# soedinglab/plass

Hardware: AMD Instinct MI355X
Metric: read-overlaps/s per assembly iteration (higher is better)
Workload: dtype u8/u64 (integer hash, byte compare; f32 ratios)

## Files before the change

### plass_amd/csrc/asm_rules.hpp

```cpp
#pragma once
#include <cmath>
#include <cstdlib>
#if defined(__HIPCC__)
#define PLASSHIP_AR_HD __host__ __device__ __forceinline__
#else
#define PLASSHIP_AR_HD static inline __attribute__((always_inline))
#endif
namespace plasship {

struct AlnCoords { int qStart, qEnd, dbStart, dbEnd; };
struct DiagSpan { bool hit = false; unsigned qo = 0, to = 0, len = 0; };

PLASSHIP_AR_HD int alnLengthOf(int qStart, int qEnd, int dbStart, int dbEnd) {
    const int aq = (qStart == -1) ? 0 : qStart, ad = (dbStart == -1) ? 0 : dbStart;
    const int dq = abs(qEnd - aq), dd = abs(dbEnd - ad);
    return (dq > dd ? dq : dd) + 1;
}
PLASSHIP_AR_HD int rawScoreOfBits(int bitScore, double ln2, double logK, double lambda) {
    return (int) (fma((double) bitScore, ln2, logK) / lambda + 0.5);
}
template <typename S> PLASSHIP_AR_HD int scorePerCol100(S score, unsigned alnLen) {
    const float scorePerCol = (float) score / (float) ((double) alnLen + 0.5);
    return (int) (scorePerCol * 100);
}
// ... 6 lines not shown
}
PLASSHIP_AR_HD AlnCoords alnOnDiagonal(int diag, int startPos, int endPos) {
    const int dist = abs(diag);
    AlnCoords c;
    if (diag >= 0) { c.qStart = startPos + dist; c.qEnd = endPos + dist; c.dbStart = startPos; c.dbEnd = endPos; }
    else { c.qStart = startPos; c.qEnd = endPos; c.dbStart = startPos + dist; c.dbEnd = endPos + dist; }
    return c;
}
PLASSHIP_AR_HD float rescoredSeqId(int ids, int qStart, int qEnd) {
    return (float) ids / ((float) qEnd - (float) qStart);
}
PLASSHIP_AR_HD bool isBranchType(int qStart, int qEnd, unsigned qLen, int dbStart, int dbEnd, unsigned dbLen) {
    const bool notBoth = !(dbStart == 0 && qStart == 0);
    const bool rightStart = dbStart == 0 && (dbEnd != (int) dbLen - 1);
    const bool leftStart = qStart == 0 && (qEnd != (int) qLen - 1);
    return (rightStart || leftStart) && notBoth;
}
PLASSHIP_AR_HD unsigned rightFragLen(unsigned tLen, int dbEnd) { return tLen - ((unsigned) dbEnd + 1); }
PLASSHIP_AR_HD bool canExtendRight(unsigned fragR, int qEnd, unsigned qLen) { return fragR > 0 && (unsigned) qEnd == (qLen - 1); }
PLASSHIP_AR_HD bool canExtendLeft(int dbStart, int dbEnd, unsigned tLen) { return dbStart > 0 && (unsigned) dbEnd == (tLen - 1); }
PLASSHIP_AR_HD bool deferredRight(unsigned fragR, int qEnd, unsigned qLen, unsigned rightOff) {
    return fragR > rightOff && (unsigned) qEnd == (qLen - 1) && rightOff > 0;
}
PLASSHIP_AR_HD bool deferredLeft(int dbStart, int dbEnd, unsigned tLen, unsigned leftOff) {
    return dbStart > (int) leftOff && (unsigned) dbEnd == (tLen - 1) && leftOff > 0;
}
PLASSHIP_AR_HD AlnCoords mirrorReverseHit(int qStart, int qEnd, int dbStart, int dbEnd, unsigned dbLen) {
    AlnCoords c;
    c.qStart = qEnd; c.qEnd = qStart;
    c.dbStart = (int) (dbLen - (unsigned) dbEnd - 1); c.dbEnd = (int) (dbLen - (unsigned) dbStart - 1);
    return c;
}

}
```

### plass_amd/csrc/assemble.hip

```cpp
#include "common.hpp"
#include "device_utils.hpp"
#include "posterior_class.hpp"
#include "ref_rules.hpp"
#include "asm_rules.hpp"
#include "host_util.hpp"
#include <algorithm>
#include <memory>
#include <cstring>

namespace plasship {

struct Item {
    uint32_t target; int32_t score; uint32_t alnLength; float seqId;
    int32_t qStart, qEnd; uint32_t qLen; int32_t dbStart, dbEnd; uint32_t dbLen;
    uint32_t state;
    uint32_t pad;
};

struct AsmArgs {
    SeqView s;
    const uint64_t *qoff; const AlnRec *recs;
    Item *items;
    const uint64_t *arenaOff;
    const uint32_t *leftCap;
// ... 1162 lines not shown
                deferred = 0;
            }
            while (deferred) {
                const int dl = __ffsll((long long) deferred) - 1;
                deferred &= deferred - 1;
                const int dqs = __shfl(xQStart, dl, G), dds = __shfl(xDbStart, dl, G);
                const char *tSeq = a.s.data + __shfl(xTOff, dl, G);
                const unsigned tLen = __shfl(xTLen, dl, G);
                const int diag = (int) ((unsigned) dqs + leftOff) - dds;
                const Rescored rs = rescoreOnDiagonalG<G>(qs, querySeqLen, tSeq, tLen, diag, smat, gl);
                nResc += (gl == 0); nRescRes += (gl == 0) ? rs.diagonalLen : 0;
                const AlnCoords c = alnOnDiagonal(diag, rs.startPos, rs.endPos);
                const float seqId = rescoredSeqId(rs.idExcl, c.qStart, c.qEnd);
                if (gl == dl) {
                    xQLen = querySeqLen; xDbLen = tLen; xAlnLen = rs.diagonalLen; xScore = scorePerCol100(rs.score, rs.diagonalLen);
                    xQStart = c.qStart; xQEnd = c.qEnd; xDbStart = c.dbStart; xDbEnd = c.dbEnd;
                    xState = (seqId >= a.seqIdThr) ? 0u : 2u;
                }
            }
            inQueue = (uint32_t) __popcll(groupBallot<G>(xState == 0));
        }
        if (couldExtend) {
            if (gl == 0) { atomicOr(&a.flags[id], 0x20u); a.newLen[id] = (uint32_t) curLen; a.newStart[id] = aoff + curStart; nExt++; }
        }
    }
    nExt = waveReduceSumU64(nExt); nResc = waveReduceSumU64(nResc); nRescRes = waveReduceSumU64(nRescRes); nAln = waveReduceSumU64(nAln); nQRes = waveReduceSumU64(nQRes);
    if (laneId() == 0) {
        if (nExt) atomicAdd(&a.stats[0], nExt); if (nResc) atomicAdd(&a.stats[1], nResc); if (nRescRes) atomicAdd(&a.stats[2], nRescRes);
        const int tier = (G <= 16) ? 0 : 1;
        if (nAln) { atomicAdd(&a.stats[3 + 3 * tier], nAln); atomicAdd(&a.stats[4 + 3 * tier], nQRes); atomicAdd(&a.stats[5 + 3 * tier], nRescRes); }
    }
}

__global__ __launch_bounds__(256) void arenaSumKernel(const AlnRec *__restrict__ recs, uint64_t nAln, uint64_t maxSeqLen, unsigned long long *__restrict__ qSum,
                                                      unsigned long long *__restrict__ qSumAa, uint32_t *__restrict__ qCan, int mirror) {
    const int lane = laneId();
    for (uint64_t i = (uint64_t) blockIdx.x * blockDim.x + threadIdx.x; i < nAln; i += (uint64_t) gridDim.x * blockDim.x) {
        const AlnRec r = recs[i];
        const uint32_t id = r.query;
        uint32_t add = 0, addAa = 0; bool can = false;
        if (r.target != id && r.accepted) {
            add = (uint32_t) r.dbLen; addAa = (uint32_t) r.dbLen / 3 + 2;
            AlnCoords c; c.qStart = r.qStart; c.qEnd = r.qEnd; c.dbStart = r.dbStart; c.dbEnd = r.dbEnd;
            if (mirror && c.qStart > c.qEnd) c = mirrorReverseHit(r.qStart, r.qEnd, r.dbStart, r.dbEnd, (unsigned) r.dbLen);
            if (isBranchType(c.qStart, c.qEnd, (unsigned) r.qLen, c.dbStart, c.dbEnd, (unsigned) r.dbLen)) {
                if (c.dbStart == 0) can = canExtendRight(rightFragLen((unsigned) r.dbLen, c.dbEnd), c.qEnd, (unsigned) r.qLen);
                else if (c.qStart == 0) can = canExtendLeft(c.dbStart, c.dbEnd, (unsigned) r.dbLen) && ((uint64_t) r.qLen + (uint64_t) c.dbStart < maxSeqLen);
            }
        }
        const unsigned long long act = __ballot(1);
        const uint32_t prevId = (uint32_t) __shfl_up((int) id, 1, 64);
        const bool head = lane == 0 || prevId != id;
        const unsigned long long heads = __ballot(head), cans = __ballot(can);
        const int segStart = 63 - __clzll((long long) (heads & (lane == 63 ? ~0ULL : ((2ULL << lane) - 1ULL))));
        const unsigned long long later = lane == 63 ? 0ULL : (heads & ~((2ULL << lane) - 1ULL));
        const int segEnd = (later ? __ffsll((long long) later) - 1 : (int) __popcll(act)) - 1;
#pragma unroll
        for (int d = 1; d < 64; d <<= 1) {
            const uint32_t t = (uint32_t) __shfl_up((int) add, d, 64), ta = (uint32_t) __shfl_up((int) addAa, d, 64);
            if (lane - d >= segStart) { add += t; addAa += ta; }
        }
        if (lane == segEnd) {
            const unsigned long long seg = (segEnd == 63 ? ~0ULL : ((2ULL << segEnd) - 1ULL)) & ~((1ULL << segStart) - 1ULL);
            if (add) atomicAdd(&qSum[id], (unsigned long long) add);
            if (qSumAa && addAa) atomicAdd(&qSumAa[id], (unsigned long long) addAa);
            if (cans & seg) atomicOr(&qCan[id], 1u);
        }
    }
}
constexpr int N_TIERS = 5;
constexpr uint8_t TIER_NARROW = 4, TIER_NONE = 0xFF;
__global__ void arenaSizeKernel(SeqView s, const uint64_t *__restrict__ qoff, const unsigned long long *__restrict__ qSum, const unsigned long long *__restrict__ qSumAa,
                                const uint32_t *__restrict__ qCan, uint32_t *__restrict__ leftCap,
                                uint64_t *__restrict__ bytes, int nuclTiers, uint64_t threadBytes,
                                uint8_t *__restrict__ tierOf,
                                const uint32_t *__restrict__ aaLen, uint32_t *__restrict__ aaLeftCap, uint64_t *__restrict__ aaBytes) {
    for (uint32_t id = blockIdx.x * blockDim.x + threadIdx.x; id < s.n; id += gridDim.x * blockDim.x) {
        int tier = -1;
        const uint64_t sum = qSum[id], sumAa = aaBytes ? qSumAa[id] : 0;
        const bool can = qCan[id] != 0;
        leftCap[id] = (uint32_t) std::min<uint64_t>(sum, 0xFFFFFFFFull);
        const uint64_t slice = (sum && can) ? (2 * sum + s.len[id] + 40) : 0;
        bytes[id] = slice;
        if (aaBytes) { aaLeftCap[id] = (uint32_t) std::min<uint64_t>(sumAa, 0xFFFFFFFFull); aaBytes[id] = (sum && can) ? (2 * sumAa + aaLen[id] + 8) : 0; }
        if (sum && can) { const uint64_t h = qoff[id + 1] - qoff[id]; tier = nuclTiers ? ((h <= 256 && slice <= threadBytes) ? 0 : 1) : (h <= 8 ? (int) TIER_NARROW : (h <= 16 ? 0 : (h <= 32 ? 1 : (h <= 64 ? 2 : 3)))); }
        tierOf[id] = (tier < 0) ? TIER_NONE : (uint8_t) tier;
    }
}
static_assert(SCAN_TILE < (1 << 12) && N_TIERS * 12 <= 64 && SCAN_BLOCK == 256, "tier counters of a tile: 12-bit fields of one 64-bit word");
__device__ __forceinline__ unsigned long long tierField(uint8_t t) { return (t < N_TIERS) ? (1ull << (12 * t)) : 0ull; }
__device__ __forceinline__ uint64_t loadTierBytes(const uint8_t *__restrict__ tierOf, uint32_t n, uint64_t base) {
    static_assert(SCAN_ITEMS == 8, "eight tier bytes per thread");
    if (base + 8 <= n) return *reinterpret_cast<const uint64_t *>(tierOf + base);
    uint64_t w = ~0ull;
    for (int k = 0; k < 8; k++) if (base + k < n) w = (w & ~(0xFFull << (8 * k))) | ((uint64_t) tierOf[base + k] << (8 * k));
    return w;
}
__global__ __launch_bounds__(SCAN_BLOCK) void tierCountKernel(const uint8_t *__restrict__ tierOf, uint32_t n, uint64_t *__restrict__ partial, uint32_t nTiles) {
    __shared__ unsigned long long wsum[SCAN_BLOCK / WAVE];
// ... 480 lines not shown
    if (al->nQueries != db->n) { setError("plasship_assemble: alignment list does not belong to the DB"); return PLASSHIP_ERR_ARG; }
    PH_ENTER(ctx);
    hipStream_t st = ctx->stream;
    const uint32_t N = (uint32_t) db->n;
    if (nucl) { const int rcS = finishSelfAlns(ctx, al); if (rcS) return rcS; }
    const uint64_t nLines = al->nSlots;
    DevBuf dLeftCap, dBytes, dArenaOff, dTmp, dItems, dFlags, dNewLen, dNewStart, dMat, dStats, dArena;
    const size_t tmpBytes = exclusiveScanTmpBytes((size_t) N + 2);
    if (dLeftCap.alloc(((size_t) N + 1) * 4) != hipSuccess || dBytes.alloc(((size_t) N + 1) * 8) != hipSuccess || dArenaOff.alloc(((size_t) N + 2) * 8) != hipSuccess ||
        dTmp.alloc(tmpBytes) != hipSuccess || dItems.alloc(std::max<uint64_t>(nLines, 1) * sizeof(Item)) != hipSuccess || dFlags.alloc(((size_t) N + 1) * 4) != hipSuccess ||
        dNewLen.alloc(((size_t) N + 1) * 4) != hipSuccess || dNewStart.alloc(((size_t) N + 1) * 8) != hipSuccess || dMat.alloc(123 * 123) != hipSuccess || dStats.alloc(128) != hipSuccess) {
        setError("plasship_assemble: out of device memory"); return PLASSHIP_ERR_DEVICE;
    }
    PH_CHECK(hipMemsetAsync(dFlags.p, 0, ((size_t) N + 1) * 4, st));
    PH_CHECK(hipMemsetAsync(dNewLen.p, 0, ((size_t) N + 1) * 4, st));
    PH_CHECK(hipMemsetAsync(dStats.p, 0, 128, st));
    PH_CHECK(hipMemcpyAsync(dMat.p, asciiSubMat(nucl), 123 * 123, hipMemcpyHostToDevice, st));
    { const int rcOL = ensureOffLen(ctx, db); if (rcOL) return rcOL; }
    const SeqView sv = db->view();
    PH_CHECK(hipEventRecord(ctx->ev[0], st));
    const uint32_t nTiles = (uint32_t) (((size_t) N + SCAN_TILE - 1) / SCAN_TILE);
    DevBuf dBigList, dMidList, dMid32List, dSmallList, dNarrowList, dTierOf, dTierPart, dAaLeftCap, dAaBytes, dAaArenaOff, dAaArena, dAaNewLen, dAaNewStart;
    if (guided && (dAaLeftCap.alloc(((size_t) N + 1) * 4) != hipSuccess || dAaBytes.alloc(((size_t) N + 1) * 8) != hipSuccess || dAaArenaOff.alloc(((size_t) N + 2) * 8) != hipSuccess ||
                   dAaNewLen.alloc(((size_t) N + 1) * 4) != hipSuccess || dAaNewStart.alloc(((size_t) N + 1) * 8) != hipSuccess)) { setError("plasship_assemble: out of device memory"); return PLASSHIP_ERR_DEVICE; }
    if (guided) PH_CHECK(hipMemsetAsync(dAaNewLen.p, 0, ((size_t) N + 1) * 4, st));
    if (dBigList.alloc(((size_t) N + 1) * 4) != hipSuccess || dMidList.alloc(((size_t) N + 1) * 4) != hipSuccess || dMid32List.alloc(((size_t) N + 1) * 4) != hipSuccess ||
        dSmallList.alloc(((size_t) N + 1) * 4) != hipSuccess || (!nucl && dNarrowList.alloc(((size_t) N + 1) * 4) != hipSuccess) || dTierOf.alloc((size_t) N + 8) != hipSuccess ||
        dTierPart.alloc(((size_t) N_TIERS * (nTiles + 1) + 1) * 8) != hipSuccess) { setError("plasship_assemble: out of device memory"); return PLASSHIP_ERR_DEVICE; }
    DevBuf dQSum, dQSumAa, dQCan;
    if (dQSum.alloc(((size_t) N + 1) * 8) != hipSuccess || dQCan.alloc(((size_t) N + 1) * 4) != hipSuccess || (guided && dQSumAa.alloc(((size_t) N + 1) * 8) != hipSuccess)) { setError("plasship_assemble: out of device memory"); return PLASSHIP_ERR_DEVICE; }
    PH_CHECK(hipMemsetAsync(dQSum.p, 0, ((size_t) N + 1) * 8, st));
    PH_CHECK(hipMemsetAsync(dQCan.p, 0, ((size_t) N + 1) * 4, st));
    if (guided) PH_CHECK(hipMemsetAsync(dQSumAa.p, 0, ((size_t) N + 1) * 8, st));
    if (nLines) hipLaunchKernelGGL(arenaSumKernel, dim3((unsigned) std::min<uint64_t>((nLines + 255) / 256, (uint64_t) ctx->numCU * 32)), dim3(256), 0, st, al->d_recs.as<AlnRec>(), (uint64_t) nLines,
                                       (uint64_t) par->max_seq_len, dQSum.as<unsigned long long>(), guided ? dQSumAa.as<unsigned long long>() : (unsigned long long *) nullptr, dQCan.as<uint32_t>(),
                                       (nucl && !guided) ? 1 : 0);
    if (N) hipLaunchKernelGGL(arenaSizeKernel, dim3(std::min<uint32_t>((N + 255) / 256, 8192)), dim3(256), 0, st, sv, al->d_qoff.as<uint64_t>(), (const unsigned long long *) dQSum.as<unsigned long long>(),
                              (const unsigned long long *) dQSumAa.as<unsigned long long>(), (const uint32_t *) dQCan.as<uint32_t>(), dLeftCap.as<uint32_t>(), dBytes.as<uint64_t>(), nucl ? 1 : 0, (uint64_t) 1 << 30,
                              dTierOf.as<uint8_t>(),
                              guided ? aaDb->d_len.as<uint32_t>() : (const uint32_t *) nullptr, dAaLeftCap.as<uint32_t>(), guided ? dAaBytes.as<uint64_t>() : (uint64_t *) nullptr);
    if (guided && exclusiveScanU64(st, dAaBytes.as<uint64_t>(), dAaArenaOff.as<uint64_t>(), N, dTmp.p, tmpBytes)) { setError("plasship_assemble: scan failed"); return PLASSHIP_ERR_DEVICE; }
    PH_CHECK(hipMemsetAsync(dTierPart.p, 0, ((size_t) N_TIERS * (nTiles + 1) + 1) * 8, st));
    if (nTiles) hipLaunchKernelGGL(tierCountKernel, dim3(nTiles), dim3(SCAN_BLOCK), 0, st, (const uint8_t *) dTierOf.as<uint8_t>(), N, dTierPart.as<uint64_t>(), nTiles);
    if (exclusiveScanU64(st, dTierPart.as<uint64_t>(), dTierPart.as<uint64_t>(), (size_t) N_TIERS * (nTiles + 1), dTmp.p, tmpBytes)) { setError("plasship_assemble: scan failed"); return PLASSHIP_ERR_DEVICE; }
    {
        TierLists tl;
        tl.list[0] = dSmallList.as<uint32_t>(); tl.list[1] = dMid32List.as<uint32_t>(); tl.list[2] = dMidList.as<uint32_t>(); tl.list[3] = dBigList.as<uint32_t>();
        tl.list[TIER_NARROW] = dNarrowList.as<uint32_t>();
        if (nTiles) hipLaunchKernelGGL(tierListKernel, dim3(nTiles), dim3(SCAN_BLOCK), 0, st, (const uint8_t *) dTierOf.as<uint8_t>(), N, (const uint64_t *) dTierPart.as<uint64_t>(), nTiles, tl);
    }
    if (exclusiveScanU64(st, dBytes.as<uint64_t>(), dArenaOff.as<uint64_t>(), N, dTmp.p, tmpBytes)) { setError("plasship_assemble: scan failed"); return PLASSHIP_ERR_DEVICE; }
    uint64_t arenaBytes = 0, aaArenaBytes = 0;
    uint64_t rowStart[N_TIERS + 1] = {};
    if (guided) PH_CHECK(hipMemcpyAsync(&aaArenaBytes, dAaArenaOff.as<uint64_t>() + N, 8, hipMemcpyDeviceToHost, st));
    PH_CHECK(hipMemcpyAsync(&arenaBytes, dArenaOff.as<uint64_t>() + N, 8, hipMemcpyDeviceToHost, st));
    PH_CHECK(hipMemcpy2DAsync(rowStart, 8, dTierPart.p, (size_t) (nTiles + 1) * 8, 8, N_TIERS + 1, hipMemcpyDeviceToHost, st));
    PH_CHECK(plasship::streamSync(st));
    uint32_t cnts[N_TIERS];
    for (int t = 0; t < N_TIERS; t++) cnts[t] = (uint32_t) (rowStart[t + 1] - rowStart[t]);
    if (dArena.alloc(arenaBytes + 64) != hipSuccess || (guided && dAaArena.alloc(aaArenaBytes + 64) != hipSuccess)) {
        size_t fr = 0, tt = 0; (void) hipMemGetInfo(&fr, &tt);
        setError("plasship_assemble: out of device memory for the extension arena (" + std::to_string(arenaBytes) + " bytes; device free " + std::to_string(fr) + " of " + std::to_string(tt) + ")"); return PLASSHIP_ERR_DEVICE;
    }
    HostEvaluer ev(nucl, db->residues);
    AsmArgs a; memset(&a, 0, sizeof(a));
    a.s = sv; a.qoff = al->d_qoff.as<uint64_t>(); a.recs = al->d_recs.as<AlnRec>(); a.items = dItems.as<Item>(); a.arenaOff = dArenaOff.as<uint64_t>();
    a.leftCap = dLeftCap.as<uint32_t>(); a.arena = dArena.as<char>(); a.flags = dFlags.as<uint32_t>(); a.newLen = dNewLen.as<uint32_t>(); a.newStart = dNewStart.as<uint64_t>();
// ... 172 lines not shown
```

### plass_amd/csrc/common.hpp

```cpp
#pragma once
#include <hip/hip_runtime.h>
#include <cstdint>
#include <cstddef>
#include <cstdio>
#include <atomic>
#include <functional>
#include <memory>
#include <mutex>
#include <string>
#include <vector>
#include "../../include/plasship.h"

namespace plasship {

void setError(const std::string &msg);
hipError_t streamSync(hipStream_t st);
}
struct plasship_seqdb; struct plasship_ctx;
namespace plasship {
int ensureOffLen(plasship_ctx *ctx, const plasship_seqdb *db);
std::string hipErrStr(hipError_t e, const char *what, const char *file, int line);

#define PH_CHECK(call)                                                                   \
    do {                                                                                 \
// ... 136 lines not shown

struct plasship_cands {
    bool reverseCapable = false;
    size_t nQueries = 0;
    uint64_t nHits = 0;
    uint64_t nNonSelf = 0;
    plasship::DevBuf d_qoff;
    plasship::DevBuf d_hits;
    std::vector<uint8_t> h_present;
};

struct plasship_clusters {
    size_t n = 0;
    uint64_t nClusters = 0;
    uint64_t dbGen = 0;
    plasship::DevBuf d_pairs;
    plasship::DevBuf d_repOf;
};

struct plasship_alns {
    size_t nQueries = 0;
    uint64_t nLines = 0;
    uint64_t nSlots = 0;
    bool sparse = false;
    mutable bool selfPending = false;
    plasship_rescore_params rsPar = {};
    bool rsSameDB = false; int rsReverseCapable = 0;
    bool nucl = false;
    bool addBacktrace = false;
    uint64_t dbResidues = 0;
    int gappedOpen = 0, gappedExtend = 0;
    plasship::DevBuf d_qoff;
    plasship::DevBuf d_recs;
    const plasship_seqdb *qdb = nullptr, *tdb = nullptr;
};

namespace plasship {
inline const plasship_comm *commOf(const plasship_ctx *ctx) { return ctx->hasComm ? &ctx->comm : nullptr; }
inline uint64_t ownedBegin(uint64_t n, int r, int world) { return ((uint64_t) r * n + (uint64_t) world - 1) / (uint64_t) world; }
int commAllgatherHost(plasship_ctx *ctx, const void *send, void *recv, uint64_t bytesPerRank);
int commAllReduceSumU64(plasship_ctx *ctx, uint64_t *v, size_t n);
int commAllReduceMaxU64(plasship_ctx *ctx, uint64_t *v, size_t n);
int commAllReduceMinU64(plasship_ctx *ctx, uint64_t *v, size_t n);
int commAgreeOk(plasship_ctx *ctx, bool ok, const char *what);
int commFinish(plasship_ctx *ctx, int rc);
int commAlltoallvRecords(plasship_ctx *ctx, const void *dSend, const uint64_t *sendCount, size_t recordBytes, DevBuf &recv,
                         uint64_t *recvTotal, uint64_t slackRecords, uint64_t *allTotal = nullptr);
int commAllgathervBytes(plasship_ctx *ctx, const void *dSend, uint64_t sendBytes, DevBuf &recv, std::vector<uint64_t> &recvBytes);
int commAllgathervBytesKnown(plasship_ctx *ctx, const void *dSend, uint64_t sendBytes, DevBuf &recv, const std::vector<uint64_t> &recvBytes);
int packedCopyOf(plasship_ctx *ctx, const plasship_seqdb *db, std::unique_ptr<plasship_seqdb> &out);
int buildOutputDB(plasship_ctx *ctx, const plasship_seqdb *db, const uint32_t *dFlags, const uint32_t *dNewLen, const uint64_t *dNewStart,
                  const char *dArena, int keepTarget, void *dTmp, size_t tmpBytes, plasship_seqdb **out,
                  const void *dExtra = nullptr, void *hExtra = nullptr, size_t extraBytes = 0, hipEvent_t doneEvent = nullptr, bool noAppend = false);
int stagedUpload(plasship_ctx *ctx, void *dDst, uint64_t total, const std::function<void(char *, uint64_t, uint64_t)> &produce,
                 uint64_t chunk = 0, const std::function<int(uint64_t)> *enqueued = nullptr);
int stagedDownload(plasship_ctx *ctx, const void *dSrc, uint64_t total, const std::function<bool(const char *, uint64_t, uint64_t)> &consume);
void *ctxPinnedTable(plasship_ctx *ctx, size_t bytes);
int stagedCopyToDevice(plasship_ctx *ctx, void *dDst, const void *hSrc, uint64_t bytes);
int stagedCopyToHost(plasship_ctx *ctx, void *hDst, const void *dSrc, uint64_t bytes);
int deviceKeysDiffer(plasship_ctx *ctx, const uint32_t *a, const uint32_t *b, size_t n, bool *differ);
int compactCsr(plasship_ctx *ctx, const char *what, const uint64_t *dInQoff, uint64_t nQ, const void *dRecs, size_t recBytes, const uint32_t *dKeep,
               uint64_t nRecs, uint64_t nKept, DevBuf &outQoff, DevBuf &outRecs);
int denseAlnsCopy(plasship_ctx *ctx, const plasship_alns *a, DevBuf &qoffBuf, DevBuf &recsBuf, const uint64_t **qoff, const AlnRec **recs);
int finishSelfAlns(plasship_ctx *ctx, const plasship_alns *a, const uint32_t *dQueryList = nullptr, uint32_t nQueryList = 0);
}
```

### plass_amd/csrc/core.hip

```cpp
#include "common.hpp"
#include "host_util.hpp"
#include "device_utils.hpp"
#include <algorithm>
#include <atomic>
#include <condition_variable>
#include <thread>
#include <memory>
#include <chrono>
#include <cstdio>
#include <cstdlib>
#include <cstring>
#include <map>
#include <mutex>
#include <numeric>
#include <unordered_map>
#include <unistd.h>

namespace plasship {
namespace {
std::mutex g_poolMu;
constexpr size_t POOL_ALIGN = 256;
struct FreeRange { size_t size; hipStream_t stream; bool mixed; };
struct Slab { char *base; size_t size; size_t used; std::map<size_t, FreeRange> free; };
struct DevicePool { std::vector<Slab> slabs; size_t total = 0; };
// ... 114 lines not shown
    std::lock_guard<std::mutex> g(g_poolMu);
    auto it = g_poolLive.find(p);
    if (it == g_poolLive.end()) { (void) hipFree(p); return; }
    const PoolLive lv = it->second;
    g_poolLive.erase(it);
    Slab &sl = g_pools[lv.device].slabs[lv.slab];
    sl.used -= lv.size;
    size_t off = lv.off, size = lv.size; hipStream_t stream = lv.stream; bool mixed = (tl_poolStream != nullptr && tl_poolStream != lv.stream);
    auto nx = sl.free.lower_bound(off);
    if (nx != sl.free.end() && off + size == nx->first) {
        if (nx->second.mixed || nx->second.stream != stream) mixed = !(nx->second.stream == nullptr && !nx->second.mixed) || mixed;
        size += nx->second.size; nx = sl.free.erase(nx);
    }
    if (nx != sl.free.begin()) {
        auto pv = std::prev(nx);
        if (pv->first + pv->second.size == off) {
            if (pv->second.mixed || pv->second.stream != stream) mixed = !(pv->second.stream == nullptr && !pv->second.mixed) || mixed;
            off = pv->first; size += pv->second.size; sl.free.erase(pv);
        }
    }
    sl.free[off] = FreeRange{size, stream, mixed};
}
void poolTrim() {
    std::lock_guard<std::mutex> g(g_poolMu);
    trimLocked(-1);
}
static thread_local std::string g_err;
int tuneInt(const char *name, int dflt) {
    char key[96]; snprintf(key, sizeof(key), "PLASSHIP_TUNE_%s", name);
    const char *e = getenv(key); const int v = e ? atoi(e) : 0;
    return v > 0 ? v : dflt;
}
static const char *const TUNE_NAMES[] = {"AGGWAVE", "AGGWAVE_CAP", "ASMQ", "ASMQ_CAP", "ROWTIER", "KMCACHE", "FORCE_LONG", "CYC_PASSES", "CYCSKIP", "SHARD_EXTRACT",
                                         "FASTA_CHUNK_MB", "DBHEAP", "DBHEAP_GB", "LAZY_SELF", "FASTQ_CHUNK_KB", "PART_BITS", "GROUP_SHAPE"};
static void reportUnknownTunes() {
    static const char PREFIX[] = "PLASSHIP_TUNE_";
    for (char **e = environ; e && *e; e++) {
        if (strncmp(*e, PREFIX, sizeof(PREFIX) - 1) != 0) continue;
        const char *x = *e + sizeof(PREFIX) - 1, *eq = strchr(x, '=');
        const std::string name(x, eq ? (size_t) (eq - x) : strlen(x));
        bool known = false;
        for (const char *k : TUNE_NAMES) known = known || name == k;
        if (!known) fprintf(stderr, "[plasship] PLASSHIP_TUNE_%s is not a switch of this build (ignored)\n", name.c_str());
    }
}
bool traceOn() { static const bool v = getenv("PLASSHIP_TRACE") != nullptr; return v; }
void setError(const std::string &msg) { g_err = msg; }
static std::atomic<unsigned long long> g_hostSyncs(0);
thread_local int tl_watchRank = -1, tl_watchWorld = 1;
thread_local const char *tl_watchLast = "none yet";
thread_local unsigned long long tl_watchCount = 0;
thread_local std::string tl_watchMsg;
void watchEnter(const plasship_ctx *ctx) {
    if (ctx && ctx->hasComm && ctx->comm.world > 1) { tl_watchRank = ctx->comm.rank; tl_watchWorld = ctx->comm.world; }
    else { tl_watchRank = -1; tl_watchWorld = 1; }
    tl_watchMsg.clear();
}
void watchCollective(const char *what) { tl_watchLast = what; tl_watchCount++; }
static double commTimeoutSeconds() { static const double v = [] { const char *e = getenv("PLASSHIP_COMM_TIMEOUT_S"); return e ? atof(e) : 300.0; }(); return v; }
hipError_t streamSync(hipStream_t st) {
    g_hostSyncs++;
    const double limit = tl_watchWorld > 1 ? commTimeoutSeconds() : 0.0;
    if (limit <= 0.0) return hipStreamSynchronize(st);
    const auto t0 = std::chrono::steady_clock::now();
    for (unsigned spins = 0;; spins++) {
        const hipError_t e = hipStreamQuery(st);
        if (e != hipErrorNotReady) return e;
// ... 476 lines not shown
```

### plass_amd/csrc/rescore.hip

```cpp
#include "common.hpp"
#include "device_utils.hpp"
#include "host_util.hpp"
#include "ref_rules.hpp"
#include "asm_rules.hpp"
#include <algorithm>
#include <memory>
#include <cfloat>
#include <cstring>

namespace plasship {

struct RescoreArgs {
    SeqView q, t;
    const uint64_t *qoff;
    const CandHit *hits;
    uint64_t nHits;
    AlnRec *out;
    const uint32_t *minScore;
    uint32_t minScoreLen;
    const signed char *mat;
    int sameDB, includeIdentity, reverseCapable;
    int covMode; float covThr;
    float seqIdThr; int alnLenThr, seqIdMode;
    double lambda, logK, ln2;
    unsigned long long *stats;
    unsigned long long *longList, *longCount;
    uint32_t shortMax;
    int mode, lazySelf;
    const uint32_t *queryList; uint32_t nQueryList;
};

constexpr int RS_BLOCK = 256;
constexpr uint32_t RS_SHORT_MAX = 768;

template <int G> __device__ __forceinline__ int groupReduceSumG(int v) {
#pragma unroll
    for (int o = G / 2; o > 0; o >>= 1) v += __shfl_xor(v, o, G);
    return v;
}
__device__ __forceinline__ uint32_t loadU32Unaligned(const char *p) { uint32_t w; __builtin_memcpy(&w, p, 4); return w; }

struct DiagScore { bool valid; unsigned score; int first, last; unsigned diagLen; int idCnt; };

template <bool REV, int G>
__device__ __forceinline__ DiagScore scoreDiagonal(const char *__restrict__ q, unsigned qLen, const char *__restrict__ t,
                                                   unsigned tLen, int diagonal, const signed char *__restrict__ smat, const unsigned char *__restrict__ comp, int sl) {
    DiagScore r; r.valid = false; r.score = 0; r.first = -1; r.last = -1; r.diagLen = 0; r.idCnt = 0;
    const DiagSpan sp = diagonalSpan(diagonal, qLen, tLen);
    if (!sp.hit) return r;
    const unsigned qo = sp.qo, to = sp.to, len = sp.len;
// ... 121 lines not shown
        if (w + stride < nWork) hitAfter = a.hits[w + stride];
    }
    for (; w < nWork; w += stride) {
        uint64_t h = (G == 1) ? w : a.longList[w];
        CandHit hit; Meta me;
        if (G == 1 && mode == 2) {
            const uint32_t qq = a.queryList[w];
            uint64_t j = a.qoff[qq]; const uint64_t j1 = a.qoff[qq + 1];
            while (j < j1 && a.out[j].btKind != ALN_SELF_PENDING) j++;
            if (j == j1) continue;
            h = j;
        }
        if (finish) {
            const AlnRec stub = a.out[h];
            if (stub.btKind != ALN_SELF_PENDING) continue;
            hit.query = stub.query; hit.target = stub.target; hit.prefScore = stub.rawScore; hit.diag16 = (uint32_t) stub.qStart;
            me = loadMeta(hit);
        } else if (G == 1) {
            hit = hitNext; me = metaNext;
            hitNext = hitAfter;
            if (w + stride < nWork) metaNext = loadMeta(hitNext);
            if (w + 2 * stride < nWork) hitAfter = a.hits[w + 2 * stride];
        } else { hit = a.hits[h]; me = loadMeta(hit); }
        const uint32_t qid = hit.query, tid = hit.target;
        const char *q = a.q.data + me.qOff;
        const unsigned qLen = me.qLen;
        const char *t = a.t.data + me.tOff;
        const unsigned tLen = me.tLen;
        if (G == 1 && !finish && a.lazySelf && qid == tid && (a.includeIdentity || a.sameDB)) {
            AlnRec stub; memset(&stub, 0, sizeof(stub));
            stub.query = qid; stub.target = tid; stub.rawScore = hit.prefScore; stub.qStart = (int32_t) hit.diag16; stub.qLen = (int) qLen; stub.dbLen = (int) tLen;
            stub.accepted = 1; stub.btKind = ALN_SELF_PENDING;
            a.out[h] = stub;
            accLocal += 1;
            continue;
        }
        if (G == 1) {
            const bool toLong = min(qLen, tLen) > a.shortMax;
            const unsigned long long m = __ballot(toLong);
            if (m) {
                const int leader = __ffsll((long long) m) - 1;
                unsigned long long basePos = 0;
                if (laneId() == leader) basePos = atomicAdd(a.longCount, (unsigned long long) __popcll(m));
                basePos = __shfl(basePos, leader, 64);
                if (toLong) a.longList[basePos + (unsigned long long) __popcll(m & ((1ULL << laneId()) - 1ULL))] = h;
            }
            if (toLong) continue;
        }
        const bool isReverse = a.reverseCapable && hit.prefScore < 0;
        const bool isIdentity = (qid == tid) && (a.includeIdentity || a.sameDB);
        AlnRec rec; memset(&rec, 0, sizeof(rec));
        rec.query = qid; rec.target = tid;
        bool accepted = false;
        if (canBeCovered(a.covThr, a.covMode, (float) qLen, (float) tLen)) {
            int bStart = -1, bEnd = -1, bDiag = 0, bIds = 0; unsigned bScore = 0, bDiagLen = 0, bDist = 0;
            const unsigned d16 = hit.diag16 & 0xFFFFu;
            const unsigned nNeg = 1 + tLen / 32768, nPos = 1 + qLen / 65536;
            const unsigned nWrap = nNeg + nPos;
            auto wrapDiag = [&](unsigned c) -> int { return c < nNeg ? (int) (d16 - (c + 1) * 65536u) : (int) ((c - nNeg) * 65536u + d16); };
            auto nextWrap = [&](unsigned c) -> unsigned {
                for (; c < nWrap; c++) { const int real = wrapDiag(c); const unsigned dist = (unsigned) abs(real); if (real >= 0 ? dist < qLen : dist < tLen) break; }
                return c;
            };
            for (unsigned c = nextWrap(0); c < nWrap; c = nextWrap(c + 1)) {
                const int real = wrapDiag(c);
                const unsigned dist = (unsigned) abs(real);
                DiagScore s = isReverse ? scoreDiagonal<true, G>(q, qLen, t, tLen, real, smat, sComp, sl) : scoreDiagonal<false, G>(q, qLen, t, tLen, real, smat, sComp, sl);
                if (s.score > bScore) { bScore = s.score; bStart = s.first; bEnd = s.last; bDiag = real; bDiagLen = s.diagLen; bDist = dist; bIds = s.idCnt; }
            }
            if (sl == 0) ovLocal += bDiagLen;
            const int distance = (int) bScore;
            const int bitScore = (int) (fma(a.lambda, (double) distance, -a.logK) / a.ln2 + 0.5);
            const int alnLen = (bEnd - bStart) + 1;
            int qS, qE, dS, dE;
            if (bDiag >= 0) { qS = bStart + (int) bDist; qE = bEnd + (int) bDist; dS = bStart; dE = bEnd; }
            else { qS = bStart; qE = bEnd; dS = bStart + (int) bDist; dE = bEnd + (int) bDist; }
            const uint32_t ms = (qLen < a.minScoreLen) ? a.minScore[qLen] : 0xFFFFFFFFu;
            const bool hasEvalue = (uint32_t) distance >= ms;
            int idCnt = bIds;
            if (bStart < 0) idCnt = isIdentity ? 1 : 0;
            float seqId = 0.0f;
            if (hasEvalue || isIdentity) seqId = computeSeqId(a.seqIdMode, idCnt, (int) qLen, (int) tLen, alnLen);
            const float queryCov = computeCov((unsigned) qS, (unsigned) qE, qLen);
            const float targetCov = computeCov((unsigned) dS, (unsigned) dE, tLen);
            if (isReverse) { qS = (int) qLen - qS - 1; qE = (int) qLen - qE - 1; }
            const bool hasCov = hasCoverage(a.covThr, a.covMode, queryCov, targetCov);
            const bool hasSeqId = (double) seqId >= (double) (a.seqIdThr - FLT_EPSILON);
            const bool hasAlnLen = alnLen >= a.alnLenThr;
            accepted = isIdentity || (hasAlnLen && hasCov && hasSeqId && hasEvalue);
            rec.bitScore = bitScore; rec.rawScore = distance; rec.seqId = seqId;
            rec.qStart = qS; rec.qEnd = qE; rec.qLen = (int) qLen; rec.dbStart = dS; rec.dbEnd = dE; rec.dbLen = (int) tLen;
            rec.alnLen = alnLen; rec.reversed = isReverse ? 1 : 0;
        }
        rec.accepted = accepted ? 1 : 0; rec.btKind = 1;
        if (sl == 0) {
            a.out[h] = rec;
            accLocal += accepted ? 1 : 0;
        }
    }
    accLocal = waveReduceSumU64(accLocal); ovLocal = waveReduceSumU64(ovLocal);
    if (laneId() == 0) {
        if (accLocal) atomicAdd(&a.stats[0], accLocal);
        if (ovLocal) atomicAdd(&a.stats[1], ovLocal);
    }
}

__global__ void acceptFlagsKernel(const AlnRec *__restrict__ recs, uint32_t *__restrict__ accept, uint64_t n) {
    for (uint64_t i = (uint64_t) blockIdx.x * blockDim.x + threadIdx.x; i < n; i += (uint64_t) gridDim.x * blockDim.x) accept[i] = recs[i].accepted ? 1u : 0u;
}
__global__ void markLengthsKernel(const uint32_t *__restrict__ len, uint32_t n, uint32_t *__restrict__ present, uint32_t cap) {
    for (uint32_t i = blockIdx.x * blockDim.x + threadIdx.x; i < n; i += gridDim.x * blockDim.x) {
        uint32_t l = len[i];
        if (l < cap) present[l] = 1;
    }
}


int denseAlnsCopy(plasship_ctx *ctx, const plasship_alns *a, DevBuf &qoffBuf, DevBuf &recsBuf, const uint64_t **qoff, const AlnRec **recs) {
    *qoff = a->d_qoff.as<uint64_t>(); *recs = a->d_recs.as<AlnRec>();
    if (!a->sparse) return PLASSHIP_OK;
    const uint64_t n = a->nSlots;
    DevBuf dAccept;
    if (dAccept.alloc(std::max<uint64_t>(n, 1) * 4) != hipSuccess) { setError("alignment list: out of device memory for the dense copy"); return PLASSHIP_ERR_DEVICE; }
    if (n) hipLaunchKernelGGL(acceptFlagsKernel, dim3((unsigned) std::min<uint64_t>((n + 255) / 256, (uint64_t) ctx->numCU * 32)), dim3(256), 0, ctx->stream, a->d_recs.as<AlnRec>(), dAccept.as<uint32_t>(), n);
    const int rc = compactCsr(ctx, "alignment list: the dense copy", a->d_qoff.as<uint64_t>(), a->nQueries, a->d_recs.p, sizeof(AlnRec), dAccept.as<uint32_t>(), n, a->nLines, qoffBuf, recsBuf);
    if (rc) return rc;
    *qoff = qoffBuf.as<uint64_t>(); *recs = recsBuf.as<AlnRec>();
    return PLASSHIP_OK;
}
// ... 48 lines not shown
    const bool nucl = qdb->dbtype == PLASSHIP_DBTYPE_NUCLEOTIDES;
    const uint64_t nHits = c->nHits;
    const uint32_t maxQLen = qdb->maxEntryLen >= 2 ? qdb->maxEntryLen - 2 : 0;

    DevBuf dPresent, dMinScore, dMat, dStats;
    const uint32_t tabLen = maxQLen + 1;
    if (dPresent.alloc((size_t) tabLen * 4) != hipSuccess || dMinScore.alloc((size_t) tabLen * 4) != hipSuccess ||
        dMat.alloc(123 * 123) != hipSuccess || dStats.alloc(16) != hipSuccess) { setError("plasship_rescore: out of device memory"); return PLASSHIP_ERR_DEVICE; }
    PH_CHECK(hipMemsetAsync(dPresent.p, 0, (size_t) tabLen * 4, ctx->stream));
    PH_CHECK(hipMemsetAsync(dStats.p, 0, 16, ctx->stream));
    if (qdb->n) hipLaunchKernelGGL(markLengthsKernel, dim3(std::min<size_t>(4096, (qdb->n + 255) / 256)), dim3(256), 0, ctx->stream,
                                   qdb->d_len.as<uint32_t>(), (uint32_t) qdb->n, dPresent.as<uint32_t>(), tabLen);
    std::vector<uint32_t> present(tabLen), minScore(tabLen, 0xFFFFFFFFu);
    PH_CHECK(hipMemcpyAsync(present.data(), dPresent.p, (size_t) tabLen * 4, hipMemcpyDeviceToHost, ctx->stream));
    PH_CHECK(plasship::streamSync(ctx->stream));
    HostEvaluer ev(nucl, tdb->residues);
    {
        const int maxEntry = nucl ? 2 : 11;
        int guess = -1;
        for (uint32_t l = 1; l < tabLen; l++)
            if (present[l]) { guess = ev.minScoreForEvalue(par->eval_thr, (int) l, maxEntry * (int) l + 1, guess); minScore[l] = (uint32_t) guess; }
    }
    PH_CHECK(hipMemcpyAsync(dMinScore.p, minScore.data(), (size_t) tabLen * 4, hipMemcpyHostToDevice, ctx->stream));
    PH_CHECK(hipMemcpyAsync(dMat.p, asciiSubMat(nucl), 123 * 123, hipMemcpyHostToDevice, ctx->stream));

    std::unique_ptr<plasship_alns> holder(new plasship_alns());
    plasship_alns *al = holder.get();
    al->nQueries = qdb->n; al->nucl = nucl; al->addBacktrace = par->add_backtrace != 0; al->dbResidues = tdb->residues;
    if (al->d_qoff.alloc((qdb->n + 1) * 8) != hipSuccess || al->d_recs.alloc(std::max<uint64_t>(nHits, 1) * sizeof(AlnRec)) != hipSuccess) {
        setError("plasship_rescore: out of device memory"); return PLASSHIP_ERR_DEVICE;
    }

    { int rcOL = ensureOffLen(ctx, qdb); if (!rcOL) rcOL = ensureOffLen(ctx, tdb); if (rcOL) return rcOL; }
    RescoreArgs a;
    a.q = qdb->view(); a.t = tdb->view(); a.qoff = c->d_qoff.as<uint64_t>(); a.hits = c->d_hits.as<CandHit>(); a.nHits = nHits;
    a.out = al->d_recs.as<AlnRec>(); a.minScore = dMinScore.as<uint32_t>(); a.minScoreLen = tabLen;
    a.mat = dMat.as<signed char>(); a.sameDB = (qdb == tdb); a.includeIdentity = par->include_identity; a.reverseCapable = c->reverseCapable;
    a.covMode = par->cov_mode; a.covThr = par->cov_thr; a.seqIdThr = par->seq_id_thr; a.alnLenThr = par->min_aln_len; a.seqIdMode = par->seq_id_mode;
    a.lambda = ev.g[0]; a.logK = ev.logK; a.ln2 = ev.ln2; a.stats = dStats.as<unsigned long long>();
    DevBuf dLongList, dLongCount;
    if (dLongList.alloc(std::max<uint64_t>(nHits, 1) * 8) != hipSuccess || dLongCount.alloc(8) != hipSuccess) { setError("plasship_rescore: out of device memory"); return PLASSHIP_ERR_DEVICE; }
    PH_CHECK(hipMemsetAsync(dLongCount.p, 0, 8, ctx->stream));
    a.longList = dLongList.as<unsigned long long>(); a.longCount = dLongCount.as<unsigned long long>();
    a.shortMax = RS_SHORT_MAX;
    a.mode = 0; a.lazySelf = tuneInt("LAZY_SELF", 1) == 1 ? 1 : 0;
    const unsigned grid = (unsigned) std::min<uint64_t>((nHits + 255) / 256 + 1, (uint64_t) ctx->numCU * (nHits > 50000000ull ? 32u : 12u));
    PH_CHECK(hipEventRecord(ctx->ev[0], ctx->stream));
    hipLaunchKernelGGL((rescoreKernel<1, 4, 0>), dim3(grid), dim3(RS_BLOCK), 0, ctx->stream, a);
    hipLaunchKernelGGL((rescoreKernel<16, 6>), dim3((unsigned) ctx->numCU * 8), dim3(RS_BLOCK), 0, ctx->stream, a);
    PH_CHECK(hipEventRecord(ctx->ev[1], ctx->stream));
    PH_CHECK(hipMemcpyAsync(al->d_qoff.p, c->d_qoff.p, (qdb->n + 1) * 8, hipMemcpyDeviceToDevice, ctx->stream));
    unsigned long long hs[2] = {0, 0};
    PH_CHECK(hipMemcpyAsync(hs, dStats.p, 16, hipMemcpyDeviceToHost, ctx->stream));
    PH_CHECK(plasship::streamSync(ctx->stream));
    PH_CHECK(hipGetLastError());
    const uint64_t nAcc = hs[0];
    al->nLines = nAcc; al->nSlots = nHits; al->sparse = true;
    al->qdb = qdb; al->tdb = tdb;
    al->selfPending = a.lazySelf != 0 && (a.sameDB || a.includeIdentity); al->rsPar = *par; al->rsSameDB = (qdb == tdb); al->rsReverseCapable = c->reverseCapable;
    if (stats) {
        stats->n_scored = nHits; stats->n_accepted = nAcc; stats->overlap_residues = hs[1];
        float ms = 0; (void) hipEventElapsedTime(&ms, ctx->ev[0], ctx->ev[1]); stats->ms_kernel = ms;
    }
    *out = holder.release();
    return PLASSHIP_OK;
}
```

Before: 744.3 million.

## Add compact per-alignment screen words to avoid full record reads in arena sum

The rescore kernel now also writes a 32-bit screen word per alignment, packing dbLen, an accepted/non-self flag, a reverse flag and precomputed extendability bits. A new arena-sum kernel walks query spans, reads only these words and finds query ids by a shuffle-based binary search over the offsets, instead of loading whole AlnRec structs. It falls back to reading the full record only in ambiguous cases (mirrored reverse hits or an undecided length limit). This trades extra writes and a device allocation during rescore for much less memory traffic during arena sizing.

```diff
diff --git a/plass_amd/csrc/asm_rules.hpp b/plass_amd/csrc/asm_rules.hpp
--- a/plass_amd/csrc/asm_rules.hpp
+++ b/plass_amd/csrc/asm_rules.hpp
@@ -62,4 +62,31 @@
     return c;
 }
 
+constexpr unsigned SCREEN_LEN_MASK = 0xFFFFFFu;
+constexpr unsigned SCREEN_COUNTS = 1u << 24;
+constexpr unsigned SCREEN_RIGHT = 1u << 25;
+constexpr unsigned SCREEN_LEFT = 1u << 26;
+constexpr unsigned SCREEN_REV = 1u << 27;
+PLASSHIP_AR_HD unsigned screenWord(bool counts, bool reversed, int qStart, int qEnd, unsigned qLen, int dbStart, int dbEnd, unsigned dbLen) {
+    unsigned w = dbLen & SCREEN_LEN_MASK;
+    if (!counts) return w;
+    w |= SCREEN_COUNTS;
+    if (reversed || qStart > qEnd) w |= SCREEN_REV;
+    if (isBranchType(qStart, qEnd, qLen, dbStart, dbEnd, dbLen)) {
+        if (dbStart == 0) { if (canExtendRight(rightFragLen(dbLen, dbEnd), qEnd, qLen)) w |= SCREEN_RIGHT; }
+        else if (qStart == 0 && canExtendLeft(dbStart, dbEnd, dbLen)) w |= (unsigned) dbStart < dbLen ? SCREEN_LEFT : (SCREEN_LEFT | SCREEN_RIGHT);
+    }
+    return w;
 }
+PLASSHIP_AR_HD int screenCanExtend(unsigned w, unsigned long long qLen, unsigned long long maxSeqLen) {
+    if (!(w & SCREEN_COUNTS)) return 0;
+    if (!(w & SCREEN_LEFT)) return (w & SCREEN_RIGHT) ? 1 : 0;
+    if (w & SCREEN_RIGHT) return -1;
+    const unsigned long long dbLen = w & SCREEN_LEN_MASK;
+    if (dbLen < 2) return -1;
+    if (qLen + dbLen - 1 < maxSeqLen) return 1;
+    if (qLen + 1 >= maxSeqLen) return 0;
+    return -1;
+}
+
+}
diff --git a/plass_amd/csrc/assemble.hip b/plass_amd/csrc/assemble.hip
--- a/plass_amd/csrc/assemble.hip
+++ b/plass_amd/csrc/assemble.hip
@@ -1218,39 +1218,74 @@
     }
 }
 
+__device__ __forceinline__ bool canStartExtension(const AlnRec &r, uint64_t maxSeqLen, int mirror) {
+    AlnCoords c; c.qStart = r.qStart; c.qEnd = r.qEnd; c.dbStart = r.dbStart; c.dbEnd = r.dbEnd;
+    if (mirror && c.qStart > c.qEnd) c = mirrorReverseHit(r.qStart, r.qEnd, r.dbStart, r.dbEnd, (unsigned) r.dbLen);
+    if (isBranchType(c.qStart, c.qEnd, (unsigned) r.qLen, c.dbStart, c.dbEnd, (unsigned) r.dbLen)) {
+        if (c.dbStart == 0) return canExtendRight(rightFragLen((unsigned) r.dbLen, c.dbEnd), c.qEnd, (unsigned) r.qLen);
+        if (c.qStart == 0) return canExtendLeft(c.dbStart, c.dbEnd, (unsigned) r.dbLen) && ((uint64_t) r.qLen + (uint64_t) c.dbStart < maxSeqLen);
+    }
+    return false;
+}
+__device__ __forceinline__ void arenaSumSegments(uint32_t id, uint32_t add, uint32_t addAa, bool can, unsigned long long act, unsigned long long *__restrict__ qSum,
+                                                 unsigned long long *__restrict__ qSumAa, uint32_t *__restrict__ qCan) {
+    const int lane = laneId();
+    const uint32_t prevId = (uint32_t) __shfl_up((int) id, 1, 64);
+    const bool head = lane == 0 || prevId != id;
+    const unsigned long long heads = __ballot(head), cans = __ballot(can);
+    const int segStart = 63 - __clzll((long long) (heads & (lane == 63 ? ~0ULL : ((2ULL << lane) - 1ULL))));
+    const unsigned long long later = lane == 63 ? 0ULL : (heads & ~((2ULL << lane) - 1ULL));
+    const int segEnd = (later ? __ffsll((long long) later) - 1 : (int) __popcll(act)) - 1;
+#pragma unroll
+    for (int d = 1; d < 64; d <<= 1) {
+        const uint32_t t = (uint32_t) __shfl_up((int) add, d, 64), ta = (uint32_t) __shfl_up((int) addAa, d, 64);
+        if (lane - d >= segStart) { add += t; addAa += ta; }
+    }
+    if (lane == segEnd) {
+        const unsigned long long seg = (segEnd == 63 ? ~0ULL : ((2ULL << segEnd) - 1ULL)) & ~((1ULL << segStart) - 1ULL);
+        if (add) atomicAdd(&qSum[id], (unsigned long long) add);
+        if (qSumAa && addAa) atomicAdd(&qSumAa[id], (unsigned long long) addAa);
+        if (cans & seg) atomicOr(&qCan[id], 1u);
+    }
+}
 __global__ __launch_bounds__(256) void arenaSumKernel(const AlnRec *__restrict__ recs, uint64_t nAln, uint64_t maxSeqLen, unsigned long long *__restrict__ qSum,
                                                       unsigned long long *__restrict__ qSumAa, uint32_t *__restrict__ qCan, int mirror) {
-    const int lane = laneId();
     for (uint64_t i = (uint64_t) blockIdx.x * blockDim.x + threadIdx.x; i < nAln; i += (uint64_t) gridDim.x * blockDim.x) {
         const AlnRec r = recs[i];
         const uint32_t id = r.query;
         uint32_t add = 0, addAa = 0; bool can = false;
         if (r.target != id && r.accepted) {
             add = (uint32_t) r.dbLen; addAa = (uint32_t) r.dbLen / 3 + 2;
-            AlnCoords c; c.qStart = r.qStart; c.qEnd = r.qEnd; c.dbStart = r.dbStart; c.dbEnd = r.dbEnd;
-            if (mirror && c.qStart > c.qEnd) c = mirrorReverseHit(r.qStart, r.qEnd, r.dbStart, r.dbEnd, (unsigned) r.dbLen);
-            if (isBranchType(c.qStart, c.qEnd, (unsigned) r.qLen, c.dbStart, c.dbEnd, (unsigned) r.dbLen)) {
-                if (c.dbStart == 0) can = canExtendRight(rightFragLen((unsigned) r.dbLen, c.dbEnd), c.qEnd, (unsigned) r.qLen);
-                else if (c.qStart == 0) can = canExtendLeft(c.dbStart, c.dbEnd, (unsigned) r.dbLen) && ((uint64_t) r.qLen + (uint64_t) c.dbStart < maxSeqLen);
-            }
-        }
-        const unsigned long long act = __ballot(1);
-        const uint32_t prevId = (uint32_t) __shfl_up((int) id, 1, 64);
-        const bool head = lane == 0 || prevId != id;
-        const unsigned long long heads = __ballot(head), cans = __ballot(can);
-        const int segStart = 63 - __clzll((long long) (heads & (lane == 63 ? ~0ULL : ((2ULL << lane) - 1ULL))));
-        const unsigned long long later = lane == 63 ? 0ULL : (heads & ~((2ULL << lane) - 1ULL));
-        const int segEnd = (later ? __ffsll((long long) later) - 1 : (int) __popcll(act)) - 1;
+            can = canStartExtension(r, maxSeqLen, mirror);
+        }
+        arenaSumSegments(id, add, addAa, can, __ballot(1), qSum, qSumAa, qCan);
+    }
+}
+__global__ __launch_bounds__(256) void arenaSumScreenKernel(const uint32_t *__restrict__ screen, const AlnRec *__restrict__ recs, const uint64_t *__restrict__ qoff,
+                                                            const uint32_t *__restrict__ qLen, uint32_t nQ, uint64_t maxSeqLen, unsigned long long *__restrict__ qSum,
+                                                            unsigned long long *__restrict__ qSumAa, uint32_t *__restrict__ qCan, int mirror) {
+    const int lane = laneId();
+    const uint32_t nSpans = (nQ + 63u) / 64u;
+    for (uint32_t sp = blockIdx.x * 4u + (threadIdx.x >> 6); sp < nSpans; sp += gridDim.x * 4u) {
+        const uint32_t q0 = sp * 64u;
+        const unsigned long long myOff = qoff[min(q0 + (uint32_t) lane, nQ)];
+        const uint64_t begin = (uint64_t) __shfl(myOff, 0, 64), end = qoff[min(q0 + 64u, nQ)];
+        for (uint64_t base = begin; base < end; base += 64) {
+            const uint64_t i = base + (uint64_t) lane;
+            const bool valid = i < end;
+            int k = 0;
 #pragma unroll
-        for (int d = 1; d < 64; d <<= 1) {
-            const uint32_t t = (uint32_t) __shfl_up((int) add, d, 64), ta = (uint32_t) __shfl_up((int) addAa, d, 64);
-            if (lane - d >= segStart) { add += t; addAa += ta; }
-        }
-        if (lane == segEnd) {
-            const unsigned long long seg = (segEnd == 63 ? ~0ULL : ((2ULL << segEnd) - 1ULL)) & ~((1ULL << segStart) - 1ULL);
-            if (add) atomicAdd(&qSum[id], (unsigned long long) add);
-            if (qSumAa && addAa) atomicAdd(&qSumAa[id], (unsigned long long) addAa);
-            if (cans & seg) atomicOr(&qCan[id], 1u);
+            for (int step = 32; step; step >>= 1) { const unsigned long long o = __shfl(myOff, k + step, 64); if (o <= i) k += step; }
+            const uint32_t id = valid ? q0 + (uint32_t) k : 0xFFFFFFFFu;
+            uint32_t add = 0, addAa = 0; bool can = false;
+            const uint32_t w = valid ? screen[i] : 0u;
+            if (w & SCREEN_COUNTS) {
+                add = w & SCREEN_LEN_MASK; addAa = add / 3 + 2;
+                int c = (mirror && (w & SCREEN_REV)) ? -1 : screenCanExtend(w, (w & SCREEN_LEFT) ? qLen[id] : 0u, maxSeqLen);
+                if (c < 0) c = canStartExtension(recs[i], maxSeqLen, mirror) ? 1 : 0;
+                can = c > 0;
+            }
+            arenaSumSegments(id, add, addAa, can, ~0ULL, qSum, qSumAa, qCan);
         }
     }
 }
@@ -1797,7 +1832,11 @@
     PH_CHECK(hipMemsetAsync(dQSum.p, 0, ((size_t) N + 1) * 8, st));
     PH_CHECK(hipMemsetAsync(dQCan.p, 0, ((size_t) N + 1) * 4, st));
     if (guided) PH_CHECK(hipMemsetAsync(dQSumAa.p, 0, ((size_t) N + 1) * 8, st));
-    if (nLines) hipLaunchKernelGGL(arenaSumKernel, dim3((unsigned) std::min<uint64_t>((nLines + 255) / 256, (uint64_t) ctx->numCU * 32)), dim3(256), 0, st, al->d_recs.as<AlnRec>(), (uint64_t) nLines,
+    const bool byScreen = al->d_screen.p != nullptr && al->qdb == db;
+    if (nLines && byScreen) hipLaunchKernelGGL(arenaSumScreenKernel, dim3(std::min<uint32_t>((N + 255) / 256, (uint32_t) ctx->numCU * 32u)), dim3(256), 0, st, (const uint32_t *) al->d_screen.as<uint32_t>(),
+                                               (const AlnRec *) al->d_recs.as<AlnRec>(), (const uint64_t *) al->d_qoff.as<uint64_t>(), (const uint32_t *) db->d_len.as<uint32_t>(), N, (uint64_t) par->max_seq_len,
+                                               dQSum.as<unsigned long long>(), guided ? dQSumAa.as<unsigned long long>() : (unsigned long long *) nullptr, dQCan.as<uint32_t>(), (nucl && !guided) ? 1 : 0);
+    else if (nLines) hipLaunchKernelGGL(arenaSumKernel, dim3((unsigned) std::min<uint64_t>((nLines + 255) / 256, (uint64_t) ctx->numCU * 32)), dim3(256), 0, st, al->d_recs.as<AlnRec>(), (uint64_t) nLines,
                                        (uint64_t) par->max_seq_len, dQSum.as<unsigned long long>(), guided ? dQSumAa.as<unsigned long long>() : (unsigned long long *) nullptr, dQCan.as<uint32_t>(),
                                        (nucl && !guided) ? 1 : 0);
     if (N) hipLaunchKernelGGL(arenaSizeKernel, dim3(std::min<uint32_t>((N + 255) / 256, 8192)), dim3(256), 0, st, sv, al->d_qoff.as<uint64_t>(), (const unsigned long long *) dQSum.as<unsigned long long>(),
diff --git a/plass_amd/csrc/common.hpp b/plass_amd/csrc/common.hpp
--- a/plass_amd/csrc/common.hpp
+++ b/plass_amd/csrc/common.hpp
@@ -192,6 +192,7 @@
     int gappedOpen = 0, gappedExtend = 0;
     plasship::DevBuf d_qoff;
     plasship::DevBuf d_recs;
+    plasship::DevBuf d_screen;
     const plasship_seqdb *qdb = nullptr, *tdb = nullptr;
 };
 
diff --git a/plass_amd/csrc/core.hip b/plass_amd/csrc/core.hip
--- a/plass_amd/csrc/core.hip
+++ b/plass_amd/csrc/core.hip
@@ -170,7 +170,7 @@
     return v > 0 ? v : dflt;
 }
 static const char *const TUNE_NAMES[] = {"AGGWAVE", "AGGWAVE_CAP", "ASMQ", "ASMQ_CAP", "ROWTIER", "KMCACHE", "FORCE_LONG", "CYC_PASSES", "CYCSKIP", "SHARD_EXTRACT",
-                                         "FASTA_CHUNK_MB", "DBHEAP", "DBHEAP_GB", "LAZY_SELF", "FASTQ_CHUNK_KB", "PART_BITS", "GROUP_SHAPE"};
+                                         "FASTA_CHUNK_MB", "DBHEAP", "DBHEAP_GB", "LAZY_SELF", "FASTQ_CHUNK_KB", "PART_BITS", "GROUP_SHAPE", "SCREEN_WORD"};
 static void reportUnknownTunes() {
     static const char PREFIX[] = "PLASSHIP_TUNE_";
     for (char **e = environ; e && *e; e++) {
diff --git a/plass_amd/csrc/rescore.hip b/plass_amd/csrc/rescore.hip
--- a/plass_amd/csrc/rescore.hip
+++ b/plass_amd/csrc/rescore.hip
@@ -16,6 +16,7 @@
     const CandHit *hits;
     uint64_t nHits;
     AlnRec *out;
+    uint32_t *screen;
     const uint32_t *minScore;
     uint32_t minScoreLen;
     const signed char *mat;
@@ -203,6 +204,7 @@
             stub.query = qid; stub.target = tid; stub.rawScore = hit.prefScore; stub.qStart = (int32_t) hit.diag16; stub.qLen = (int) qLen; stub.dbLen = (int) tLen;
             stub.accepted = 1; stub.btKind = ALN_SELF_PENDING;
             a.out[h] = stub;
+            if (a.screen) a.screen[h] = screenWord(false, false, 0, 0, qLen, 0, 0, tLen);
             accLocal += 1;
             continue;
         }
@@ -266,6 +268,7 @@
         rec.accepted = accepted ? 1 : 0; rec.btKind = 1;
         if (sl == 0) {
             a.out[h] = rec;
+            if (a.screen) a.screen[h] = screenWord(accepted && qid != tid, isReverse, rec.qStart, rec.qEnd, qLen, rec.dbStart, rec.dbEnd, tLen);
             accLocal += accepted ? 1 : 0;
         }
     }
@@ -380,9 +383,11 @@
     }
 
     { int rcOL = ensureOffLen(ctx, qdb); if (!rcOL) rcOL = ensureOffLen(ctx, tdb); if (rcOL) return rcOL; }
+    const bool screenWords = tuneInt("SCREEN_WORD", 1) == 1;
+    if (screenWords && al->d_screen.alloc(std::max<uint64_t>(nHits, 1) * 4) != hipSuccess) { setError("plasship_rescore: out of device memory"); return PLASSHIP_ERR_DEVICE; }
     RescoreArgs a;
     a.q = qdb->view(); a.t = tdb->view(); a.qoff = c->d_qoff.as<uint64_t>(); a.hits = c->d_hits.as<CandHit>(); a.nHits = nHits;
-    a.out = al->d_recs.as<AlnRec>(); a.minScore = dMinScore.as<uint32_t>(); a.minScoreLen = tabLen;
+    a.out = al->d_recs.as<AlnRec>(); a.screen = screenWords ? al->d_screen.as<uint32_t>() : nullptr; a.minScore = dMinScore.as<uint32_t>(); a.minScoreLen = tabLen;
     a.mat = dMat.as<signed char>(); a.sameDB = (qdb == tdb); a.includeIdentity = par->include_identity; a.reverseCapable = c->reverseCapable;
     a.covMode = par->cov_mode; a.covThr = par->cov_thr; a.seqIdThr = par->seq_id_thr; a.alnLenThr = par->min_aln_len; a.seqIdMode = par->seq_id_mode;
     a.lambda = ev.g[0]; a.logK = ev.logK; a.ln2 = ev.ln2; a.stats = dStats.as<unsigned long long>();
```

Result: no change. 748.2 million (median of 6 runs) (+0.5%).
